# HaydenFaulkner/Tennis

Hardware: AMD Instinct MI355X
Metric: frames/sec DenseNet-121 224x224 feature-extract (higher is better)
Workload: dtype f16

## Files before the change

tennis_amd/csrc/api.hip:

```cpp
#include <cmath>
#include <cstdlib>
#include <cstring>
#include <map>
#include <string>
#include <vector>

#include "common.h"
#include "linear.h"
#include "rnn.h"
#include "train.h"

bool dense_layer_big_supported(int H, int W);

static thread_local std::string g_err;
void tn_set_error(const std::string &msg) { g_err = msg; }
extern "C" const char *tn_last_error(void) { return g_err.c_str(); }
extern "C" int tn_version(void) { return 100; }

extern "C" int tn_ctx_create(int device, void *stream, int own_stream, tn_ctx **out) {
  TN_REQUIRE(out != nullptr, "tn_ctx_create: out is null");
  int n = 0;
  TN_HIP_CHECK(hipGetDeviceCount(&n));
  TN_REQUIRE(device >= 0 && device < n, "tn_ctx_create: no such device");
  TN_ON_DEVICE(device);
// ... 136 lines not shown
          const int n = nf * 16 + (l & 15), slot = (l >> 4) * 8 + j, kx = (slot >> 2) - (zero_first ? 1 : 0), c = slot & 3;
          float v = 0.f;
          if (kx >= 0 && kx < 7 && c < 3) v = w[(((size_t)n * 3 + c) * 7 + ky) * 7 + kx];
          p[(((size_t)ky * 4 + nf) * 64 + l) * 8 + j] = (f16)v;
        }
  return p;
}

struct EventTimer {
  bool on = false;
  hipStream_t s = nullptr;
  struct Rec { hipEvent_t a, b; int fam; };
  std::vector<Rec> recs;
  std::vector<tn_kernel_stat> fams;
  int family(const char *name) {
    for (size_t i = 0; i < fams.size(); ++i)
      if (!strcmp(fams[i].name, name)) return (int)i;
    tn_kernel_stat st;
    memset(&st, 0, sizeof(st));
    strncpy(st.name, name, sizeof(st.name) - 1);
    fams.push_back(st);
    return (int)fams.size() - 1;
  }
  void begin(const char *name, double flops, double bytes) {
    if (!on) return;
    Rec r;
    r.fam = family(name);
    (void)hipEventCreate(&r.a);
    (void)hipEventCreate(&r.b);
    fams[r.fam].launches += 1;
    fams[r.fam].flops += flops;
    fams[r.fam].bytes += bytes;
    (void)hipEventRecord(r.a, s);
    recs.push_back(r);
  }
  void end() {
    if (!on) return;
    (void)hipEventRecord(recs.back().b, s);
  }
  void finish() {
    if (!on) return;
    (void)hipStreamSynchronize(s);
    for (auto &r : recs) {
      float ms = 0.f;
      (void)hipEventElapsedTime(&ms, r.a, r.b);
      fams[r.fam].ms += ms;
      (void)hipEventDestroy(r.a);
      (void)hipEventDestroy(r.b);
    }
    recs.clear();
  }
};

}

struct tn_encoder {
  tn_ctx *ctx;
  DevPool pool;
  int H, W, maxB, feat_dim;
  int Hs, Ws;
  int Hb[4], Wb[4];
  int Cin[4], Cb[4];
  int PH, PW;
  f16 *stem_wp, *stem_wp_zf, *stem_wp_zf_lo = nullptr;
  float *stem_scale, *stem_shift, *stem_shift_u8;
  float *stem_floor = nullptr;
  std::vector<float> stem_centre;
  std::vector<float> calib_centre;
  struct DenseLayer { float *s1, *t1; f16 *w1; float *s2, *t2; f16 *w3p; int cin; f16 *w1s = nullptr, *w3s = nullptr; };
  std::vector<DenseLayer> layers[4];
  struct Trans { float *s, *t; f16 *w; int cin, cout; f16 *wfrag = nullptr; } trans[3];
  float *head_s, *head_t;
  float *zeros128 = nullptr;
  f16 *stem_out, *bott, *blockbuf[4];
  float *head32 = nullptr;
  size_t workspace_bytes;
  int last_batch;
  bool fuse, split;
  int nsplit;
  int dl_variant;
  bool chain;
  bool exact = false;
  bool strip = true;
  int strip_min_batch = 64;
  DenseLayerDev *chain_dev[4] = {nullptr, nullptr, nullptr, nullptr};
  float *calib_dev = nullptr;
  double *calib_scratch = nullptr;
  float *ones128 = nullptr;
  bool block7 = true;
  DenseBlock7Args b7[4] = {};
  bool block14 = true;
  DenseBlock14Args b14[4] = {};
  f16 *b14_scratch[4] = {nullptr, nullptr, nullptr, nullptr};
  bool block28 = false;
  DenseBlock28Args b28[4] = {};
  f16 *b28_scratch[4] = {nullptr, nullptr, nullptr, nullptr};
  hipStream_t side[4];
  hipEvent_t ev_in, ev_done[2][4];
  bool pipelined = false;
  bool last_interleaved = false;
  int last_ws0 = 0;
  bool interleave = false;
  long calls = 0;
  int split_of[2] = {0, 0};
  int split_batch = 0;
};

static const int kBlockCfg[4] = {6, 12, 24, 16};

extern "C" int tn_densenet121_create(tn_ctx *ctx, const tn_param *params, int n_params, const char *prefix_c,
                                     int height, int width, int max_batch, tn_encoder **out) {
  return tn_densenet121_create_ex(ctx, params, n_params, prefix_c, height, width, max_batch, 0, out);
}

extern "C" int tn_densenet121_create_ex(tn_ctx *ctx, const tn_param *params, int n_params, const char *prefix_c,
                                        int height, int width, int max_batch, int flags, tn_encoder **out) {
  TN_REQUIRE(ctx && params && out && prefix_c, "tn_densenet121_create: null argument");
  TN_REQUIRE((flags & ~TN_ENC_EXACT_WEIGHTS) == 0, "tn_densenet121_create_ex: unknown flag");
  TN_REQUIRE(max_batch > 0, "tn_densenet121_create: max_batch must be positive");
  TN_REQUIRE(height >= 224 && width >= 224 && height <= 1024 && width <= 1024,
             "tn_densenet121_create: input size must be in [224,1024] (AvgPool2D(7) needs a >=7x7 final map)");
  TN_ON_DEVICE(ctx->device);
  const std::string pre(prefix_c);
  ParamMap pm(params, n_params);
  tn_encoder *e = new tn_encoder();
  e->ctx = ctx;
  e->H = height; e->W = width; e->maxB = max_batch; e->last_batch = 0;
  e->fuse = getenv("TN_NO_FUSE") == nullptr;
  e->split = getenv("TN_NO_SPLIT") == nullptr;
  e->nsplit = getenv("TN_SPLIT") ? atoi(getenv("TN_SPLIT")) : 2;
  if (e->nsplit != 4) e->nsplit = 2;
  e->block7 = getenv("TN_NO_BLOCK7") == nullptr;
  e->block14 = getenv("TN_NO_BLOCK14") == nullptr;
  e->block28 = getenv("TN_BLOCK28") != nullptr && atoi(getenv("TN_BLOCK28")) != 0;
  e->chain = getenv("TN_NO_CHAIN") == nullptr;
  e->dl_variant = getenv("TN_DL_VARIANT") ? atoi(getenv("TN_DL_VARIANT")) : 0;
  e->exact = (flags & TN_ENC_EXACT_WEIGHTS) != 0;
  e->strip = getenv("TN_NO_STRIP") == nullptr && !e->exact && e->fuse;
  if (getenv("TN_STRIP_MIN_BATCH")) e->strip_min_batch = atoi(getenv("TN_STRIP_MIN_BATCH"));
  for (int i = 0; i < 4; ++i) {
    if (hipStreamCreateWithFlags(&e->side[i], hipStreamNonBlocking) != hipSuccess ||
        hipEventCreateWithFlags(&e->ev_done[0][i], hipEventDisableTiming) != hipSuccess ||
        hipEventCreateWithFlags(&e->ev_done[1][i], hipEventDisableTiming) != hipSuccess) {
      tn_set_error("could not create the side streams");
      delete e;
      return TN_ERR_HIP;
    }
  }
  if (hipEventCreateWithFlags(&e->ev_in, hipEventDisableTiming) != hipSuccess) { tn_set_error("hipEventCreate failed"); delete e; return TN_ERR_HIP; }
  e->Hs = (height + 6 - 7) / 2 + 1; e->Ws = (width + 6 - 7) / 2 + 1;
  int h = (e->Hs + 2 - 3) / 2 + 1, w = (e->Ws + 2 - 3) / 2 + 1, c = 64;
  for (int b = 0; b < 4; ++b) {
    e->Hb[b] = h; e->Wb[b] = w; e->Cin[b] = c; e->Cb[b] = c + 32 * kBlockCfg[b];
    c = e->Cb[b] / 2; h /= 2; w /= 2;
  }
  e->PH = e->Hb[3] / 7; e->PW = e->Wb[3] / 7;
  e->feat_dim = e->Cb[3] * e->PH * e->PW;
  auto fail = [&](int code) { e->pool.release(); delete e; return code; };
  if (e->PH < 1 || e->PW < 1) { tn_set_error("input too small for AvgPool2D(7)"); return fail(TN_ERR_INVALID); }
  if (e->Wb[0] > 240) { tn_set_error("input too wide for the conv3x3 LDS tile"); return fail(TN_ERR_INVALID); }
  if (e->exact) {
    const bool ok = e->fuse && (e->dl_variant & ~256) == 0;
    if (!ok) { tn_set_error("TN_ENC_EXACT_WEIGHTS needs the default kernels (no TN_NO_FUSE, no TN_DL_VARIANT)"); return fail(TN_ERR_INVALID); }
  }

  std::vector<float> s, t;
  e->stem_centre.assign(64, 0.f);
  if (getenv("TN_NO_STEM_CENTRE") == nullptr) {
    std::vector<double> acc(64, 0.0);
    int cnt = 0;
    for (int l = 0; l <= kBlockCfg[0]; ++l) {
      const std::string bn = l < kBlockCfg[0] ? pre + "stage1_batchnorm" + std::to_string(2 * l) : pre + "batchnorm1";
      const float *mu = pm.get(bn + "_running_mean", l < kBlockCfg[0] ? 64 + 32 * l : 64 + 32 * kBlockCfg[0]);
      if (!mu) return fail(TN_ERR_MISSING);
      for (int c = 0; c < 64; ++c) acc[c] += mu[c];
      ++cnt;
    }
    for (int c = 0; c < 64; ++c) {
      const float m = (float)(acc[c] / cnt);
      e->stem_centre[c] = std::isfinite(m) ? m : 0.f;
    }
  }
  auto centre_shift = [&](std::vector<float> &sc, std::vector<float> &sh) {
    for (int c = 0; c < 64; ++c) sh[c] = (float)((double)sh[c] + (double)sc[c] * (double)e->stem_centre[c]);
  };
  {
    const float *w0 = pm.get(pre + "conv0_weight", 64 * 3 * 7 * 7);
    if (!w0 || !fold_bn(pm, pre + "batchnorm0", 64, s, t)) return fail(TN_ERR_MISSING);
    std::vector<float> w0s((size_t)64 * 3 * 49), tu(64);
    for (int n = 0; n < 64; ++n) {
      double bias = 0.0;
      for (int c = 0; c < 3; ++c)
        for (int k = 0; k < 49; ++k) {
          const size_t i = ((size_t)n * 3 + c) * 49 + k;
          w0s[i] = w0[i] * stem_wfactor(c);
          bias -= (double)(float)(f16)w0s[i] * stem_pad(c);
        }
      s[n] = (float)((double)s[n] / kStemWScale);
      tu[n] = (float)((double)t[n] + (double)s[n] * bias);
    }
    e->stem_wp = e->pool.upload(pack_stem(w0s.data(), false));
    e->stem_wp_zf = e->pool.upload(pack_stem(w0s.data(), true));
    if (e->exact) {
      std::vector<float> lo(w0s.size());
      for (int n = 0; n < 64; ++n) {
        double bias = 0.0;
        for (int c = 0; c < 3; ++c)
          for (int k = 0; k < 49; ++k) {
            const size_t i = ((size_t)n * 3 + c) * 49 + k;
            const float hi = (float)(f16)w0s[i];
            lo[i] = w0s[i] - hi;
            bias -= ((double)hi + (double)(float)(f16)lo[i]) * stem_pad(c);
          }
        tu[n] = (float)((double)t[n] + (double)s[n] * bias);
      }
      e->stem_wp_zf_lo = e->pool.upload(pack_stem(lo.data(), true));
    }
    std::vector<float> fl(64);
    for (int n = 0; n < 64; ++n) {
      t[n] = (float)((double)t[n] - (double)e->stem_centre[n]);
      tu[n] = (float)((double)tu[n] - (double)e->stem_centre[n]);
      fl[n] = -e->stem_centre[n];
    }
    e->stem_scale = e->pool.upload(s);
    e->stem_shift = e->pool.upload(t);
    e->stem_shift_u8 = e->pool.upload(tu);
    e->stem_floor = e->pool.upload(fl);
  }
  e->zeros128 = e->pool.upload(std::vector<float>(128, 0.0f));
  e->ones128 = e->pool.upload(std::vector<float>(128, 1.0f));
  int outer = 1;
  for (int b = 0; b < 4; ++b) {
    const std::string sp = pre + "stage" + std::to_string(b + 1) + "_";
    const bool pack14 = e->fuse && e->block14 && !e->exact && dense_block14_supported(e->Hb[b], e->Wb[b], e->Cin[b], kBlockCfg[b]);
    const bool pack28 = e->fuse && e->block28 && !e->exact && dense_block28_supported(e->Hb[b], e->Wb[b], e->Cin[b], kBlockCfg[b]);
    const bool pack7 = (e->fuse && e->block7 && !e->exact && dense_block7_supported(e->Hb[b], e->Wb[b], e->Cin[b], kBlockCfg[b])) || pack14 || pack28;
    std::vector<std::vector<float>> h7[4];
    std::vector<const float *> h7w3;
    for (int l = 0; l < kBlockCfg[b]; ++l) {
      tn_encoder::DenseLayer L;
      L.cin = e->Cin[b] + 32 * l;
      const float *w1 = pm.get(sp + "conv" + std::to_string(2 * l) + "_weight", (int64_t)128 * L.cin);
      const float *w3 = pm.get(sp + "conv" + std::to_string(2 * l + 1) + "_weight", 32 * 128 * 9);
      if (!w1 || !w3) return fail(TN_ERR_MISSING);
      if (!fold_bn(pm, sp + "batchnorm" + std::to_string(2 * l), L.cin, s, t)) return fail(TN_ERR_MISSING);
      if (b == 0) centre_shift(s, t);
      std::vector<float> sw1(L.cin), tc1(L.cin);
      bn_relu_clamp_fold(std::vector<float>(s).data(), std::vector<float>(t).data(), L.cin, s.data(), t.data(), sw1.data(), tc1.data());
      L.s1 = e->pool.upload(s); L.t1 = e->pool.upload(t);
      if (b == 0)
        for (int c = 0; c < 64; ++c) e->calib_centre.push_back(s[c] != t[c] ? e->stem_centre[c] : 0.f);
      std::vector<float> x0(L.cin);
      for (int k = 0; k < L.cin; ++k) x0[k] = std::fmin(std::fmax(0.f, s[k]), t[k]);
      if (pack7) { h7[1].push_back(s); h7[2].push_back(t); h7w3.push_back(w3); }
      if (!fold_bn(pm, sp + "batchnorm" + std::to_string(2 * l + 1), 128, s, t)) return fail(TN_ERR_MISSING);
      std::vector<float> w1f((size_t)128 * L.cin);
      bool in_range = true;
      for (int n = 0; n < 128; ++n) {
        double bias = 0.0, corr = 0.0;
        for (int k = 0; k < L.cin; ++k) {
          const float wf = s[n] * sw1[k] * w1[(size_t)n * L.cin + k];
          w1f[(size_t)n * L.cin + k] = wf;
          in_range = in_range && std::fabs(wf) <= 65504.0f;
          bias += (double)w1[(size_t)n * L.cin + k] * ((double)tc1[k] + (double)sw1[k] * (double)x0[k]);
          if (x0[k] != 0.f) {
            const float hi = (float)(f16)wf;
            const double weff = e->exact ? (double)hi + (double)(float)(f16)(wf - hi) : (double)hi;
            corr += weff * (double)x0[k];
          }
        }
        t[n] = (float)((double)t[n] + (double)s[n] * bias - corr);
      }
      if (!in_range) { tn_set_error("a 1x1 weight leaves the fp16 range once its BatchNorm scales are folded in (" + sp + "conv" + std::to_string(2 * l) + ")"); return fail(TN_ERR_INVALID); }
      if (e->exact) {
        const bool tile = dense_layer_supported(e->Hb[b], e->Wb[b]) && L.cin <= dense_layer_kmax(e->Wb[b]);
        const int bk = !tile ? 64 : (e->Hb[b] == 14 || e->Hb[b] == 7) ? 64 : 32;
        L.w1 = e->pool.upload(split_hi_lo_rows(w1f.data(), 128, L.cin, (L.cin + bk - 1) / bk * bk));
      } else {
        L.w1 = e->pool.upload(to_f16(w1f.data(), (size_t)128 * L.cin));
      }
      if (pack7) { h7[0].push_back(w1f); h7[3].push_back(t); }
      if (e->strip && dense_strip_supported(e->Hb[b], e->Wb[b], L.cin)) L.w1s = e->pool.upload(pack_w1_strip(w1f.data(), L.cin, t.data()));
      L.s2 = e->pool.upload(std::vector<float>(128, 1.0f)); L.t2 = e->pool.upload(t);
      if (e->exact) {
        std::vector<float> hi(32 * 128 * 9), lo(32 * 128 * 9);
        for (size_t i = 0; i < hi.size(); ++i) {
          hi[i] = (float)(f16)w3[i];
          lo[i] = w3[i] - hi[i];
        }
        std::vector<f16> img = pack_conv3x3(hi.data());
        const std::vector<f16> img_lo = pack_conv3x3(lo.data());
        img.insert(img.end(), img_lo.begin(), img_lo.end());
        L.w3p = e->pool.upload(img);
      } else {
        L.w3p = e->pool.upload(pack_conv3x3(w3));
      }
      if (L.w1s) L.w3s = e->pool.upload(pack_w3_strip(w3));
      e->layers[b].push_back(L);
    }
    if (pack14) {
      std::vector<Block14Layer> bl;
      for (int l = 0; l < kBlockCfg[b]; ++l)
        bl.push_back(Block14Layer{h7[0][l].data(), h7w3[l], h7[1][l].data(), h7[2][l].data(), h7[3][l].data()});
      DenseBlock14Args &a14 = e->b14[b];
      a14.stream = e->pool.upload(pack_block14(bl, e->Cin[b]));
      a14.total_units = dense_block14_units(e->Cin[b], kBlockCfg[b]);
      a14.ldc = e->Cb[b]; a14.K0 = e->Cin[b]; a14.nl = kBlockCfg[b];
    } else if (pack28) {
      std::vector<Block14Layer> bl;
      for (int l = 0; l < kBlockCfg[b]; ++l)
        bl.push_back(Block14Layer{h7[0][l].data(), h7w3[l], h7[1][l].data(), h7[2][l].data(), h7[3][l].data()});
      DenseBlock28Args &a28 = e->b28[b];
      a28.stream = e->pool.upload(pack_block28(bl, e->Cin[b]));
      a28.total_units = dense_block28_units(e->Cin[b], kBlockCfg[b]);
      a28.ldc = e->Cb[b]; a28.K0 = e->Cin[b]; a28.nl = kBlockCfg[b];
    } else if (pack7) {
      std::vector<Block7Layer> bl;
      for (int l = 0; l < kBlockCfg[b]; ++l)
        bl.push_back(Block7Layer{h7[0][l].data(), h7w3[l], h7[1][l].data(), h7[2][l].data(), h7[3][l].data()});
      const Block7Image img = pack_block7(bl, e->Cin[b]);
      DenseBlock7Args &a7 = e->b7[b];
      a7.wa = e->pool.upload(img.wa); a7.wb = e->pool.upload(img.wb); a7.tab = e->pool.upload(img.tab);
      for (int w = 0; w < 4; ++w) { a7.a_off[w] = img.a_off[w]; a7.b_off[w] = img.b_off[w]; }
      a7.ldc = e->Cb[b]; a7.K0 = e->Cin[b]; a7.nl = kBlockCfg[b];
    }
    {
      std::vector<DenseLayerDev> cd;
      for (auto &L : e->layers[b]) cd.push_back(DenseLayerDev{L.s1, L.t1, L.w1, L.s2, L.t2, L.w3p});
      e->chain_dev[b] = e->pool.upload(cd);
    }
    if (b < 3) {
      auto &T = e->trans[b];
      T.cin = e->Cb[b]; T.cout = e->Cb[b] / 2;
      const float *wt = pm.get(pre + "conv" + std::to_string(outer) + "_weight", (int64_t)T.cout * T.cin);
      if (!wt || !fold_bn(pm, pre + "batchnorm" + std::to_string(outer), T.cin, s, t)) return fail(TN_ERR_MISSING);
      if (b == 0) centre_shift(s, t);
      T.s = e->pool.upload(s); T.t = e->pool.upload(t);
      T.w = e->exact ? e->pool.upload(split_hi_lo_rows(wt, T.cout, T.cin, T.cin))
                     : e->pool.upload(to_f16(wt, (size_t)T.cout * T.cin));
      if (!e->exact && (T.cout == 512 || T.cout == 256) && T.cin % 128 == 0) {
        const std::vector<f16> wh = to_f16(wt, (size_t)T.cout * T.cin);
        T.wfrag = e->pool.upload(pack_trans_frags(wh.data(), T.cout, T.cin));
      }
      ++outer;
    }
  }
  if (!fold_bn(pm, pre + "batchnorm" + std::to_string(outer), e->Cb[3], s, t)) return fail(TN_ERR_MISSING);
  e->head_s = e->pool.upload(s); e->head_t = e->pool.upload(t);

  const size_t weights_bytes = e->pool.bytes;
  e->interleave = getenv("TN_NO_INTERLEAVE") == nullptr && e->split && max_batch >= 64;
  const size_t B = (size_t)max_batch * (e->interleave ? 2 : 1);
  e->stem_out = (f16 *)e->pool.alloc(B * e->Hs * e->Ws * 64 * sizeof(f16));
  e->bott = (f16 *)e->pool.alloc(B * e->Hb[0] * e->Wb[0] * 128 * sizeof(f16));
  for (int b = 0; b < 4; ++b)
    e->blockbuf[b] = (f16 *)e->pool.alloc(B * e->Hb[b] * e->Wb[b] * e->Cb[b] * sizeof(f16));
  if (e->b7[3].wa) e->head32 = (float *)e->pool.alloc(B * e->Hb[3] * e->Wb[3] * e->Cb[3] * sizeof(float));
  for (int b = 0; b < 4; ++b)
    if (e->b14[b].stream) e->b14_scratch[b] = (f16 *)e->pool.alloc(B * dense_block14_scratch_halfs() * sizeof(f16));
  for (int b = 0; b < 4; ++b)
    if (e->b28[b].stream) e->b28_scratch[b] = (f16 *)e->pool.alloc(B * dense_block28_scratch_halfs() * sizeof(f16));
  e->workspace_bytes = e->pool.bytes - weights_bytes;
  if (e->pool.failed) { tn_set_error("device allocation failed"); return fail(TN_ERR_NOMEM); }
  for (int b = 0; b < 4; ++b)
    if (e->b14[b].stream && (hipMemset(e->blockbuf[b], 0, B * e->Hb[b] * e->Wb[b] * e->Cb[b] * sizeof(f16)) != hipSuccess ||
// ... 653 lines not shown
```

tennis_amd/csrc/dense_strip.hip:

```cpp
#include <array>
#include <vector>

#include "common.h"

int launch_dense_strip_w56(const DenseStripArgs &a, hipStream_t s);
int launch_dense_strip_w28(const DenseStripArgs &a, hipStream_t s);
int launch_dense_strip_w128(const DenseStripArgs &a, hipStream_t s);
int launch_dense_strip_w64(const DenseStripArgs &a, hipStream_t s);

bool dense_strip_supported(int H, int W, int K) {
  return H == W && (W == 56 || W == 28 || W == 128 || W == 64) && K % 32 == 0 && K >= 64 && K <= (W == 128 ? 288 : 320);
}

int launch_dense_strip(const DenseStripArgs &a, hipStream_t s) {
  TN_REQUIRE(dense_strip_supported(a.H, a.W, a.K), "dense_strip: unsupported geometry");
  TN_REQUIRE(a.buf && a.s1 && a.t1 && a.w1s && a.w3s, "dense_strip: null operand");
  TN_REQUIRE(a.ldc % 64 == 0 && a.K + 32 <= a.ldc, "dense_strip: bad channel geometry");
  if (a.W == 56) return launch_dense_strip_w56(a, s);
  if (a.W == 128) return launch_dense_strip_w128(a, s);
  if (a.W == 64) return launch_dense_strip_w64(a, s);
  return launch_dense_strip_w28(a, s);
}

std::vector<f16> pack_w1_strip(const float *w, int K, const float *shift) {
  const int ks = K / 32, kq = K / 16, nsu = (ks + 1) / 2;
  std::vector<f16> p((size_t)(kq + 1) * 4 * 64 * 8, (f16)0.f);
  for (int mb = 0; mb < 4; ++mb)
    for (int l = 0; l < 32; ++l) {
      f16 *d = &p[(((size_t)kq * 4 + mb) * 64 + l) * 8];
      const float t = shift[32 * mb + l];
      d[0] = (f16)t;
      d[1] = (f16)(t - (float)d[0]);
      d[2] = (f16)1.f;
    }
  for (int q = 0; q < kq; ++q) {
    const int u = q >> 2, i = q & 3;
    const bool half = (ks & 1) && u == nsu - 1;
    for (int mb = 0; mb < 4; ++mb)
      for (int l = 0; l < 64; ++l)
        for (int j = 0; j < 8; ++j) {
          const int c = (half ? 64 * u + 16 * (l >> 5) : 64 * u + 32 * (l >> 5)) + 8 * i + j;
          p[(((size_t)q * 4 + mb) * 64 + l) * 8 + j] = (f16)w[(size_t)(32 * mb + (l & 31)) * K + c];
        }
  }
  return p;
}

std::vector<f16> pack_w3_strip(const float *w) {
  constexpr int kW3Bytes = 3 * 8 * 3 * 1024;
  std::vector<f16> p((size_t)kW3Bytes / 2);
  for (int dy = 0; dy < 3; ++dy)
    for (int t = 0; t < 8; ++t)
      for (int dx = 0; dx < 3; ++dx)
        for (int l = 0; l < 64; ++l)
          for (int j = 0; j < 8; ++j) {
            const int m = l & 31, o = 16 * ((m >> 2) & 1) + (m & 3) + 4 * (m >> 3);
            const int c = 16 * t + 8 * (j >> 2) + 4 * (l >> 5) + (j & 3);
            p[(((((size_t)dy * 8 + t) * 3 + dx) * 64) + l) * 8 + j] = (f16)w[(((size_t)o * 128 + c) * 3 + dy) * 3 + dx];
          }
  return p;
}
```

tennis_amd/csrc/dense_strip_impl.h:

```cpp
#include <array>
#include <type_traits>

#pragma once
#include "common.h"

#ifndef TN_DS_EXP
#define TN_DS_EXP 0
#endif

namespace {

typedef unsigned u32x4 __attribute__((ext_vector_type(4)));
typedef _Float16 h2_t __attribute__((ext_vector_type(2)));

constexpr int kW3Bytes = 3 * 8 * 3 * 1024;

template <int W, int KS>
struct DSGeom {
  static constexpr int NPAIR = (W + 27) / 28;
  static constexpr int ROWS = W == 56 ? 28 : W == 28 ? 7 : W / 4;
  static constexpr int NCHUNK = W / ROWS;
  static constexpr int NITEM = NPAIR * NCHUNK, WGS = NITEM / 4;
  static constexpr int KQ = 2 * KS;
  static constexpr int NSU = (KS + 1) / 2;
  static constexpr int W1OFF = kW3Bytes;
  static constexpr int T1OFF = W1OFF + (KQ + 1) * 4096;
  static constexpr int LDS_BYTES = T1OFF + KS * 32 * 4;
  static_assert(W % ROWS == 0 && NITEM % 4 == 0 && ROWS >= 4, "strip geometry");
  static_assert(NSU <= 5, "the activation ring holds five super-steps");
  static_assert(LDS_BYTES <= 160 * 1024, "weights do not fit LDS");
};

#define TN_WIN_BASE 160
#define TN_WIN_CLOBBER                                                                                                              \
  "a160", "a161", "a162", "a163", "a164", "a165", "a166", "a167", "a168", "a169", "a170", "a171", "a172", "a173", "a174", "a175",   \
  "a176", "a177", "a178", "a179", "a180", "a181", "a182", "a183", "a184", "a185", "a186", "a187", "a188", "a189", "a190", "a191",   \
  "a192", "a193", "a194", "a195", "a196", "a197", "a198", "a199", "a200", "a201", "a202", "a203", "a204", "a205", "a206", "a207",   \
  "a208", "a209", "a210", "a211", "a212", "a213", "a214", "a215", "a216", "a217", "a218", "a219", "a220", "a221", "a222", "a223",   \
  "a224", "a225", "a226", "a227", "a228", "a229", "a230", "a231", "a232", "a233", "a234", "a235", "a236", "a237", "a238", "a239",   \
  "a240", "a241", "a242", "a243", "a244", "a245", "a246", "a247", "a248", "a249", "a250", "a251", "a252", "a253", "a254", "a255"
constexpr int win_reg(int prow, int t) { return TN_WIN_BASE + 32 * prow + 4 * t; }
#define TN_WIN_FENCE() asm volatile("" ::: TN_WIN_CLOBBER)

template <int PROW, int T>
__device__ __forceinline__ void win_write(const unsigned v0, const unsigned v1, const unsigned v2, const unsigned v3) {
  constexpr int B = win_reg(PROW, T);
  asm volatile("v_accvgpr_write_b32 a%c4, %0\n\tv_accvgpr_write_b32 a%c5, %1\n\tv_accvgpr_write_b32 a%c6, %2\n\tv_accvgpr_write_b32 a%c7, %3"
               :: "v"(v0), "v"(v1), "v"(v2), "v"(v3), "n"(B), "n"(B + 1), "n"(B + 2), "n"(B + 3) : TN_WIN_CLOBBER);
}
template <int R>
__device__ __forceinline__ void win_zero_reg() {
  asm volatile("v_accvgpr_write_b32 a%c0, 0" :: "n"(R) : TN_WIN_CLOBBER);
}
template <int PROW>
__device__ __forceinline__ void win_zero() {
  [&]<int... I>(std::integer_sequence<int, I...>) { (win_zero_reg<win_reg(PROW, 0) + I>(), ...); }(std::make_integer_sequence<int, 32>{});
  asm volatile("s_nop 1");
}
template <bool FIRST, int PROW, int T>
__device__ __forceinline__ void mfma32_win(f32x16 &d, const u32x4 a) {
  constexpr int B0 = win_reg(PROW, T);
  if constexpr (FIRST)
    asm volatile("v_mfma_f32_32x32x16_f16 %0, %1, a[%c2:%c3], 0" : "=&a"(d) : "v"(a), "n"(B0), "n"(B0 + 3));
  else
    asm volatile("v_mfma_f32_32x32x16_f16 %0, %1, a[%c2:%c3], %0" : "+a"(d) : "v"(a), "n"(B0), "n"(B0 + 3));
}
template <int PROW, int T>
__device__ __forceinline__ void mfma32_win_last3(f32x16 &d0, f32x16 &d1, f32x16 &d2, const u32x4 a0, const u32x4 a1, const u32x4 a2) {
  constexpr int B0 = win_reg(PROW, T);
  asm volatile("v_mfma_f32_32x32x16_f16 %0, %3, a[%c6:%c7], %0\n\tv_mfma_f32_32x32x16_f16 %1, %4, a[%c6:%c7], %1\n\t"
               "v_mfma_f32_32x32x16_f16 %2, %5, a[%c6:%c7], %2\n\ts_nop 15\n\ts_nop 3"
               : "+a"(d0), "+a"(d1), "+a"(d2) : "v"(a0), "v"(a1), "v"(a2), "n"(B0), "n"(B0 + 3));
}
__device__ __forceinline__ f32x16 mfma32(const u32x4 a, const u32x4 b, const f32x16 c) {
  return __builtin_amdgcn_mfma_f32_32x32x16_f16(__builtin_bit_cast(f16x8, a), __builtin_bit_cast(f16x8, b), c, 0, 0, 0);
}

template <int CTRL>
__device__ __forceinline__ float dpp_f32(float v) {
  return __builtin_bit_cast(float, __builtin_amdgcn_update_dpp(0, __builtin_bit_cast(int, v), CTRL, 0xf, 0xf, true));
}

#define TN_INL __attribute__((always_inline))
template <int N, typename F>
__device__ __forceinline__ void static_for(F &&f) {
  [&]<int... I>(std::integer_sequence<int, I...>) TN_INL { (f(std::integral_constant<int, I>{}), ...); }(std::make_integer_sequence<int, N>{});
}
template <int V>
using ic = std::integral_constant<int, V>;

#define TN_SB() __builtin_amdgcn_sched_barrier(0)

__device__ __forceinline__ void dma16(const void *gsrc, unsigned lds_dst) {
  unsigned keep;
  asm volatile("s_mov_b32 %0, m0\n\ts_mov_b32 m0, %2\n\ts_nop 0\n\tglobal_load_lds_dwordx4 %1, off\n\ts_mov_b32 m0, %0"
               : "=&s"(keep)
               : "v"(gsrc), "s"(lds_dst)
               : "memory");
}

struct PItem { int kind, q, j; };
template <int KS>
struct PList { PItem it[7 * 2 * KS + 8]; int n; };
template <int KS>
constexpr PList<KS> make_pl() {
  constexpr int KQ = 2 * KS, NSU = (KS + 1) / 2;
  constexpr bool ODD = (KS & 1) != 0;
  PList<KS> l{};
  int n = 0;
  for (int c = 0; c < 3 && c < KQ; ++c) l.it[n++] = PItem{1, c, 0};
  for (int q = 0; q < KQ; ++q) {
    for (int j = 0; j < 4; ++j) l.it[n++] = PItem{2, q, j};
    if (q + 3 < KQ) l.it[n++] = PItem{1, q + 3, 0};
    const int u = q >> 2;
    const bool half = ODD && u == NSU - 1;
    if (half ? (q & 3) == 1 : (q & 3) == 3)
      for (int i = 0; i < (half ? 2 : 4); ++i) l.it[n++] = PItem{3, u, i};
  }
  l.n = n;
  return l;
}
template <int KS>
inline constexpr PList<KS> kPL = make_pl<KS>();
template <int KS>
constexpr PItem pl_at(int idx) { return idx >= 0 && idx < kPL<KS>.n ? kPL<KS>.it[idx] : PItem{0, 0, 0}; }
template <int KS>
constexpr int pl_len() { return kPL<KS>.n; }
constexpr int kPLB = 30;
constexpr int kXN = 8;
struct ASlot { int pl0, npl, epb0, nepb; };
template <int N> struct ASched { ASlot s[N]; };
template <int KS>
constexpr auto make_a_sched() {
  constexpr int KQ = 2 * KS, NA = 4 * (KQ + 1), NPL = pl_len<KS>();
  ASched<NA> r{};
  int bn3[KQ + 1] = {};
  for (int i = 0; i < NPL; ++i)
    if (kPL<KS>.it[i].kind == 2 && kPL<KS>.it[i].j == 3) bn3[kPL<KS>.it[i].q] = i;
  int pos = NPL < kPLB ? NPL : kPLB, epb = 0;
  for (int i = 0; i < NA; ++i) {
    const int qn = i / 4 + 1, rem = 3 - i % 4;
    const int need_end = qn < KQ ? bn3[qn] + 1 : 0;
    const int left = NA - i, total = (NPL - pos) + (24 - epb);
    int quota = (total + left - 1) / left;
    int must = need_end - rem - pos;
    if (must < 0) must = 0;
    if (must > NPL - pos) must = NPL - pos;
    int npl = must;
    if (quota < npl) quota = npl;
    int ne = 24 - epb < quota - npl ? 24 - epb : quota - npl;
    const int more = NPL - pos - npl < quota - npl - ne ? NPL - pos - npl : quota - npl - ne;
    npl += more;
    r.s[i] = ASlot{pos, npl, epb, ne};
    pos += npl;
    epb += ne;
  }
  return r;
}
template <int KS>
constexpr bool a_sched_complete() {
  constexpr int KQ = 2 * KS, NA = 4 * (KQ + 1);
  constexpr auto sa = make_a_sched<KS>();
  int npl = pl_len<KS>() < kPLB ? pl_len<KS>() : kPLB, nepb = 0;
  for (int i = 0; i < NA; ++i) { npl += sa.s[i].npl; nepb += sa.s[i].nepb; }
  return npl == pl_len<KS>() && nepb == 24;
}

template <int W, int KS>
__global__ __launch_bounds__(256) __attribute__((amdgpu_waves_per_eu(1, 1))) void dense_strip_kernel(DenseStripArgs a) {
  using G = DSGeom<W, KS>;
  constexpr int H = W, NSU = G::NSU, K = KS * 32, KQ = G::KQ, ROWS = G::ROWS;
  constexpr bool ODD = (KS & 1) != 0;
  constexpr int XN = kXN, NPL = pl_len<KS>(), PLB = NPL < kPLB ? NPL : kPLB;
  static_assert(a_sched_complete<KS>(), "1x1 slot schedule leaves work unassigned");
  extern __shared__ __attribute__((aligned(16))) unsigned char smem[];
  const int tid = threadIdx.x;
  if (a.ts && tid == 0) {
    a.ts[(size_t)blockIdx.x * 128 + 127] = __builtin_amdgcn_s_memtime();
    a.ts[(size_t)blockIdx.x * 128 + 126] = __builtin_amdgcn_s_memrealtime();
  }

  {
    typedef __attribute__((address_space(3))) void *lptr_t;
    const unsigned lds0 = __builtin_amdgcn_readfirstlane((unsigned)(size_t)(lptr_t)smem);
    const int wv = __builtin_amdgcn_readfirstlane(tid >> 6), ln = tid & 63;
    constexpr int P3 = kW3Bytes / 1024, P1 = (KQ + 1) * 4;
    const unsigned char *g3 = (const unsigned char *)a.w3s + ln * 16, *g1 = (const unsigned char *)a.w1s + ln * 16;
    for (int p = wv; p < P3; p += 4) dma16(g3 + p * 1024, lds0 + p * 1024);
    for (int p = wv; p < P1; p += 4) dma16(g1 + p * 1024, lds0 + G::W1OFF + p * 1024);
    f16 *t1 = (f16 *)(smem + G::T1OFF);
    for (int i = tid; i < K; i += 256) {
      t1[i] = (f16)a.s1[i];
      t1[K + i] = (f16)a.t1[i];
    }
    asm volatile("s_waitcnt vmcnt(0)" ::: "memory");
  }
  __syncthreads();

  const int lane = tid & 63;
  const int wid = __builtin_amdgcn_readfirstlane(tid >> 6);
  const int n = lane & 31, h = lane >> 5;
  const int item = (int)(blockIdx.x % G::WGS) * 4 + wid;
  const int pair = item % G::NPAIR, part = item / G::NPAIR;
  const int r_lo = part * ROWS, r_hi = r_lo + ROWS;
  const int x = 14 * (2 * pair + (n >> 4)) - 1 + (n & 15);
  const bool xvalid = x >= 0 && x < W;
  const int xc = x < 0 ? 0 : (x >= W ? W - 1 : x);
  const int ldc = a.ldc;
  const unsigned rowpitch = (unsigned)W * ldc * 2;
  unsigned char *fb = (unsigned char *)(a.buf + (size_t)(blockIdx.x / G::WGS) * H * W * ldc);
  const unsigned colb = (unsigned)xc * ldc * 2 + 64 * h;
  const unsigned colh = (unsigned)xc * ldc * 2 + 32 * h;
  const bool store_ok = (n & 15) >= 1 && (n & 15) <= 14 && xvalid;
  const unsigned outb = (unsigned)xc * ldc * 2 + K * 2 + 32 * h;
  const __amdgpu_buffer_rsrc_t orsrc = __builtin_amdgcn_make_buffer_rsrc(fb, 0, (int)((unsigned)H * rowpitch), 0x00020000);

  const unsigned char *w1l = smem + G::W1OFF + lane * 16;
  const unsigned char *w3l = smem + lane * 16;
  const f16 *tab1 = (const f16 *)(smem + G::T1OFF);
  const u32x4 xb_shift = {h == 0 ? 0x3c003c00u : 0u, (h == 0 && !xvalid) ? 0x0000fb53u : 0u, 0u, 0u};

  u32x4 ring[5][4];
  f32x16 acc[4];
  u32x4 wa[2][4];
  u32x4 xb[XN];
  u32x4 cs[3], ct[3];
  u32x4 w3f[2][3];
  f32x16 bacc[3];
  unsigned e_pk[4];
  float o_c[2], o_l[2], o_r[2];
  unsigned o_pk[8];

  auto rowbase = [&](int y) TN_INL {
    const int yc = y < 0 ? 0 : (y >= H ? H - 1 : y);
    return fb + (unsigned)yc * rowpitch;
  };
  auto ld_item = [&](auto u_tag, auto i_tag, int y) TN_INL {
    constexpr int U = decltype(u_tag)::value, I = decltype(i_tag)::value;
    constexpr bool HALF = ODD && U == NSU - 1;
    if ((TN_DS_EXP & 1) && y > r_lo + 1) return;
    if constexpr (HALF) ring[U][I] = *(const u32x4 *)(rowbase(y) + colh + 128 * U + 16 * I);
    else ring[U][I] = *(const u32x4 *)(rowbase(y) + colb + 128 * U + 16 * I);
  };
  auto consts_item = [&](auto q_tag) TN_INL {
    constexpr int Q = decltype(q_tag)::value;
    constexpr int U = Q >> 2, I = Q & 3;
    constexpr bool HALF = ODD && U == NSU - 1;
    const int c0 = (HALF ? 64 * U + 16 * h : 64 * U + 32 * h) + 8 * I;
    cs[Q % 3] = *(const u32x4 *)(tab1 + c0);
    ct[Q % 3] = *(const u32x4 *)(tab1 + K + c0);
  };
  auto bn_item = [&](auto q_tag, auto j_tag) TN_INL {
    constexpr int Q = decltype(q_tag)::value, J = decltype(j_tag)::value;
    const unsigned in = ring[Q >> 2][Q & 3][J];
    const unsigned sc = cs[Q % 3][J], sh = ct[Q % 3][J];
    unsigned o;
    asm("v_pk_max_f16 %0, %1, %2\n\tv_pk_min_f16 %0, %0, %3" : "=&v"(o) : "v"(in), "v"(sc), "v"(sh));
    xb[Q % XN][J] = o;
  };
  auto pl_item = [&](auto idx_tag, int ybn) TN_INL {
    constexpr PItem it = pl_at<KS>(decltype(idx_tag)::value);
    if constexpr (it.kind == 1) consts_item(ic<it.q>{});
    else if constexpr (it.kind == 2) bn_item(ic<it.q>{}, ic<it.j>{});
    else if constexpr (it.kind == 3) ld_item(ic<it.q>{}, ic<it.j>{}, ybn + 1);
  };
  auto wa_item = [&](auto q_tag, auto mb_tag) TN_INL {
    constexpr int Q = decltype(q_tag)::value, MB = decltype(mb_tag)::value;
    if ((TN_DS_EXP & 16) && Q >= 2) return;
    wa[Q & 1][MB] = *(const u32x4 *)(w1l + (Q * 4 + MB) * 1024);
  };
  auto wa_group = [&](auto q_tag) TN_INL { static_for<4>([&](auto mb_tag) TN_INL { wa_item(q_tag, mb_tag); }); };
  auto prologue_exposed = [&](int ybn) TN_INL {
    wa_group(ic<0>{});
    wa_group(ic<1>{});
    static_for<PLB>([&](auto i_tag) TN_INL { pl_item(i_tag, ybn); });
    TN_SB();
  };

  auto epa_item = [&](auto prow_tag, auto e_tag) TN_INL {
    constexpr int PROW = decltype(prow_tag)::value, E = decltype(e_tag)::value;
    constexpr int T = E / 5, I = E % 5, MB = T >> 1, R0 = 8 * (T & 1);
    unsigned (&epk)[4] = e_pk;
    f32x16 (&accr)[4] = acc;
    if constexpr (I < 4) {
      const float a0 = accr[MB][R0 + 2 * I], a1 = accr[MB][R0 + 2 * I + 1];
      asm("v_cvt_pk_f16_f32 %0, %1, %2\n\tv_pk_max_f16 %0, %0, 0" : "=v"(epk[I]) : "v"(a0), "v"(a1));
    } else {
      win_write<PROW, T>(epk[0], epk[1], epk[2], epk[3]);
    }
  };
  auto epilogue_a_exposed = [&](auto prow_tag) TN_INL {
    static_for<40>([&](auto e_tag) TN_INL { epa_item(prow_tag, e_tag); });
    TN_SB();
  };
  auto epb_item = [&](auto i_tag, unsigned off) TN_INL {
    constexpr int I = decltype(i_tag)::value, P = I / 3, PART = I % 3;
    if constexpr (PART == 0) {
      o_c[0] = bacc[1][2 * P]; o_c[1] = bacc[1][2 * P + 1];
      o_l[0] = bacc[0][2 * P]; o_l[1] = bacc[0][2 * P + 1];
    } else if constexpr (PART == 1) {
      o_c[0] += dpp_f32<0x111>(o_l[0]);
      o_c[1] += dpp_f32<0x111>(o_l[1]);
      o_r[0] = bacc[2][2 * P]; o_r[1] = bacc[2][2 * P + 1];
    } else {
      o_c[0] += dpp_f32<0x101>(o_r[0]);
      o_c[1] += dpp_f32<0x101>(o_r[1]);
      const h2_t p = {(f16)o_c[0], (f16)o_c[1]};
      o_pk[P] = __builtin_bit_cast(unsigned, p);
      if constexpr (P == 3 || P == 7) {
        const u32x4 o = {o_pk[P - 3], o_pk[P - 2], o_pk[P - 1], o_pk[P]};
        __builtin_amdgcn_raw_buffer_store_b128(o, orsrc, off + (P == 7 ? 16 : 0), 0, 0);
      }
    }
  };
  auto out_offset = [&](int yo, bool valid) TN_INL { return (valid && store_ok) ? outb + (unsigned)yo * rowpitch : 0x80000000u; };
  auto bacc_ready = [&]() TN_INL {
    f32x16 (&b)[3] = bacc;
    asm volatile("s_nop 15\n\ts_nop 3" : "+a"(b[0]), "+a"(b[1]), "+a"(b[2]));
  };
  auto epilogue_b_exposed = [&](int yo) TN_INL {
    bacc_ready();
    const unsigned off = out_offset(yo, true);
    static_for<24>([&](auto i_tag) TN_INL { epb_item(i_tag, off); TN_SB(); });
  };
  auto w3_item = [&](auto s_tag, auto dx_tag) TN_INL {
    constexpr int S = decltype(s_tag)::value, DX = decltype(dx_tag)::value;
    if ((TN_DS_EXP & 8) && S >= 2) return;
    w3f[S & 1][DX] = *(const u32x4 *)(w3l + (S * 3 + DX) * 1024);
  };

  auto phase_a = [&](int yb, int yo_prev, bool prev_valid) TN_INL {
    constexpr auto SA = make_a_sched<KS>();
    bacc_ready();
    const unsigned off_prev = out_offset(yo_prev, prev_valid);
    static_for<KQ + 1>([&](auto q_tag) TN_INL {
      constexpr int Q = decltype(q_tag)::value;
      static_for<4>([&](auto mb_tag) TN_INL {
        constexpr int MB = decltype(mb_tag)::value, SL = 4 * Q + MB;
        if constexpr (MB == 0) {
          u32x4 (&w)[4] = wa[Q & 1];
          asm volatile("" :: "v"(w[0]), "v"(w[1]), "v"(w[2]), "v"(w[3]));
        }
        if constexpr (Q == 0) {
          f32x16 z;
#pragma unroll
          for (int i = 0; i < 16; ++i) z[i] = 0.f;
          acc[MB] = mfma32(wa[0][MB], xb[0], z);
        } else if constexpr (Q == KQ) {
          acc[MB] = mfma32(wa[Q & 1][MB], xb_shift, acc[MB]);
        } else {
          acc[MB] = mfma32(wa[Q & 1][MB], xb[Q % XN], acc[MB]);
        }
        if constexpr (Q + 2 < KQ + 1) wa_item(ic<Q + 2>{}, mb_tag);
        constexpr ASlot sl = SA.s[SL];
        static_for<sl.npl>([&](auto k_tag) TN_INL { pl_item(ic<sl.pl0 + decltype(k_tag)::value>{}, yb); });
        static_for<sl.nepb>([&](auto k_tag) TN_INL { epb_item(ic<sl.epb0 + decltype(k_tag)::value>{}, off_prev); });
        TN_WIN_FENCE();
        TN_SB();
      });
    });
  };

  auto phase_b = [&](auto rot_tag, auto epa_tag, int ybn) TN_INL {
    constexpr int ROT = decltype(rot_tag)::value;
    constexpr bool HAS_EPA = decltype(epa_tag)::value != 0;
    static_for<72>([&](auto e_tag) TN_INL {
      constexpr int E = decltype(e_tag)::value;
      constexpr int S = E / 3, DX = E % 3, DY = S / 8, T = S % 8;
      constexpr int PROW = (ROT + 1 + DY) % 3;
      if constexpr (DX == 0) {
        u32x4 (&w)[3] = w3f[S & 1];
        asm volatile("" :: "v"(w[0]), "v"(w[1]), "v"(w[2]));
      }
      if constexpr (S < 23) mfma32_win<S == 0, PROW, T>(bacc[DX], w3f[S & 1][DX]);
      else if constexpr (DX == 2) mfma32_win_last3<PROW, T>(bacc[0], bacc[1], bacc[2], w3f[S & 1][0], w3f[S & 1][1], w3f[S & 1][2]);
      if constexpr (S + 2 < 24) w3_item(ic<S + 2>{}, ic<DX>{});
      if constexpr (E < 40) {
        if constexpr (HAS_EPA) epa_item(rot_tag, e_tag);
      } else if constexpr (E < 42) {
        wa_group(ic<E - 40>{});
      } else if constexpr (E - 42 < PLB) {
        pl_item(ic<E - 42>{}, ybn);
      }
      TN_WIN_FENCE();
      TN_SB();
    });
  };
  auto load_w3_first = [&]() TN_INL { static_for<6>([&](auto i_tag) TN_INL { w3_item(ic<decltype(i_tag)::value / 3>{}, ic<decltype(i_tag)::value % 3>{}); }); };

  int nstamp = 0;
  auto stamp = [&]() TN_INL {
    if (a.ts && wid == 0 && nstamp < 125) {
      if (lane == 0) a.ts[(size_t)blockIdx.x * 128 + nstamp] = __builtin_amdgcn_s_memtime();
      ++nstamp;
    }
  };
  auto row_event = [&](auto rot_tag, int yb, bool prev_valid) TN_INL {
    stamp();
    if (!(TN_DS_EXP & 4)) phase_a(yb, yb - 2, prev_valid);
    load_w3_first();
    TN_SB();
    stamp();
    if (!(TN_DS_EXP & 2)) phase_b(rot_tag, ic<1>{}, yb + 1);
  };

  {
    f32x16 z;
#pragma unroll
    for (int i = 0; i < 16; ++i) z[i] = 0.f;
    bacc[0] = z; bacc[1] = z; bacc[2] = z;
  }
  stamp();
  const int yfirst = r_lo > 0 ? r_lo - 1 : 0;
  static_for<NSU>([&](auto u_tag) TN_INL {
    constexpr bool HALF = ODD && decltype(u_tag)::value == NSU - 1;
    static_for<(HALF ? 2 : 4)>([&](auto i_tag) TN_INL { ring[decltype(u_tag)::value][decltype(i_tag)::value] =
        *(const u32x4 *)(rowbase(yfirst) + (HALF ? colh : colb) + 128 * decltype(u_tag)::value + 16 * decltype(i_tag)::value); });
  });
  if (r_lo > 0) {
    prologue_exposed(r_lo - 1);
    phase_a(r_lo - 1, 0, false);
    epilogue_a_exposed(ic<0>{});
  } else {
    win_zero<0>();
  }
  prologue_exposed(r_lo);
  phase_a(r_lo, 0, false);
  epilogue_a_exposed(ic<1>{});
  prologue_exposed(r_lo + 1);
  stamp();
  int yb = r_lo + 1;
  for (; yb + 2 < r_hi; yb += 3) {
    row_event(ic<2>{}, yb, yb > r_lo + 1);
    row_event(ic<0>{}, yb + 1, true);
    row_event(ic<1>{}, yb + 2, true);
  }
  constexpr int NREM = (ROWS - 1) % 3;
  if constexpr (NREM >= 1) { row_event(ic<2>{}, yb, yb > r_lo + 1); ++yb; }
  if constexpr (NREM >= 2) { row_event(ic<0>{}, yb, true); ++yb; }
  constexpr int ROTL = (ROWS + 1) % 3;
  if (r_hi < H) {
    row_event(ic<ROTL>{}, r_hi, true);
  } else {
    epilogue_b_exposed(r_hi - 2);
    win_zero<ROTL>();
    load_w3_first();
    TN_SB();
    phase_b(ic<ROTL>{}, ic<0>{}, r_hi);
  }
  stamp();
  epilogue_b_exposed(r_hi - 1);
  stamp();
  if (a.ts && wid == 0 && lane == 0) a.ts[(size_t)blockIdx.x * 128 + 125] = __builtin_amdgcn_s_memrealtime();
}

template <int W, int KS>
int launch_strip(const DenseStripArgs &a, hipStream_t s) {
  using G = DSGeom<W, KS>;
  TN_SET_ATTR_ONCE_PER_DEVICE(TN_HIP_CHECK(hipFuncSetAttribute((const void *)dense_strip_kernel<W, KS>, hipFuncAttributeMaxDynamicSharedMemorySize, G::LDS_BYTES)));
  hipLaunchKernelGGL((dense_strip_kernel<W, KS>), dim3(a.B * G::WGS), dim3(256), G::LDS_BYTES, s, a);
  TN_HIP_CHECK(hipGetLastError());
  return TN_OK;
}

template <int W>
int launch_strip_w(const DenseStripArgs &a, hipStream_t s) {
  switch (a.K / 32) {
    case 2: return launch_strip<W, 2>(a, s);
    case 3: return launch_strip<W, 3>(a, s);
    case 4: return launch_strip<W, 4>(a, s);
    case 5: return launch_strip<W, 5>(a, s);
    case 6: return launch_strip<W, 6>(a, s);
    case 7: return launch_strip<W, 7>(a, s);
    case 8: return launch_strip<W, 8>(a, s);
    case 9: return launch_strip<W, 9>(a, s);
    case 10:
      if constexpr (W != 128) return launch_strip<W, 10>(a, s);
      break;
  }
  TN_REQUIRE(false, "dense_strip: K out of range");
}

}
```

Measured before the change: 134,200.

## Extend fused strip dense-layer kernel to wider 28x28 inputs via global-memory weight tail

Lets the fused 1x1+3x3 strip kernel handle 28x28 dense layers with up to 480 input channels. When the 1x1 weights no longer fit in LDS, the first k-steps stay LDS-resident and the rest are streamed from global memory with buffer loads. The activation ring is re-indexed modulo a shorter depth, and a third weight register slot is added for small tails. Layers that previously fell back to the slower unfused path now run fused, at the cost of more global weight traffic and register pressure in those instances.

```diff
diff --git a/tennis_amd/csrc/api.hip b/tennis_amd/csrc/api.hip
--- a/tennis_amd/csrc/api.hip
+++ b/tennis_amd/csrc/api.hip
@@ -242,6 +242,7 @@
   bool chain;
   bool exact = false;
   bool strip = true;
+  int strip_kmax = 480;
   int strip_min_batch = 64;
   DenseLayerDev *chain_dev[4] = {nullptr, nullptr, nullptr, nullptr};
   float *calib_dev = nullptr;
@@ -298,6 +299,7 @@
   e->exact = (flags & TN_ENC_EXACT_WEIGHTS) != 0;
   e->strip = getenv("TN_NO_STRIP") == nullptr && !e->exact && e->fuse;
   if (getenv("TN_STRIP_MIN_BATCH")) e->strip_min_batch = atoi(getenv("TN_STRIP_MIN_BATCH"));
+  if (getenv("TN_STRIP_KMAX")) e->strip_kmax = atoi(getenv("TN_STRIP_KMAX"));
   for (int i = 0; i < 4; ++i) {
     if (hipStreamCreateWithFlags(&e->side[i], hipStreamNonBlocking) != hipSuccess ||
         hipEventCreateWithFlags(&e->ev_done[0][i], hipEventDisableTiming) != hipSuccess ||
@@ -440,7 +442,7 @@
         L.w1 = e->pool.upload(to_f16(w1f.data(), (size_t)128 * L.cin));
       }
       if (pack7) { h7[0].push_back(w1f); h7[3].push_back(t); }
-      if (e->strip && dense_strip_supported(e->Hb[b], e->Wb[b], L.cin)) L.w1s = e->pool.upload(pack_w1_strip(w1f.data(), L.cin, t.data()));
+      if (e->strip && L.cin <= e->strip_kmax && dense_strip_supported(e->Hb[b], e->Wb[b], L.cin)) L.w1s = e->pool.upload(pack_w1_strip(w1f.data(), L.cin, t.data()));
       L.s2 = e->pool.upload(std::vector<float>(128, 1.0f)); L.t2 = e->pool.upload(t);
       if (e->exact) {
         std::vector<float> hi(32 * 128 * 9), lo(32 * 128 * 9);
diff --git a/tennis_amd/csrc/dense_strip.hip b/tennis_amd/csrc/dense_strip.hip
--- a/tennis_amd/csrc/dense_strip.hip
+++ b/tennis_amd/csrc/dense_strip.hip
@@ -5,11 +5,13 @@
 
 int launch_dense_strip_w56(const DenseStripArgs &a, hipStream_t s);
 int launch_dense_strip_w28(const DenseStripArgs &a, hipStream_t s);
+int launch_dense_strip_w28_tail(const DenseStripArgs &a, hipStream_t s);
 int launch_dense_strip_w128(const DenseStripArgs &a, hipStream_t s);
 int launch_dense_strip_w64(const DenseStripArgs &a, hipStream_t s);
 
 bool dense_strip_supported(int H, int W, int K) {
-  return H == W && (W == 56 || W == 28 || W == 128 || W == 64) && K % 32 == 0 && K >= 64 && K <= (W == 128 ? 288 : 320);
+  return H == W && (W == 56 || W == 28 || W == 128 || W == 64) && K % 32 == 0 && K >= 64 &&
+         K <= (W == 128 ? 288 : W == 28 ? 480 : 320);
 }
 
 int launch_dense_strip(const DenseStripArgs &a, hipStream_t s) {
@@ -19,7 +21,7 @@
   if (a.W == 56) return launch_dense_strip_w56(a, s);
   if (a.W == 128) return launch_dense_strip_w128(a, s);
   if (a.W == 64) return launch_dense_strip_w64(a, s);
-  return launch_dense_strip_w28(a, s);
+  return a.K > 320 ? launch_dense_strip_w28_tail(a, s) : launch_dense_strip_w28(a, s);
 }
 
 std::vector<f16> pack_w1_strip(const float *w, int K, const float *shift) {
diff --git a/tennis_amd/csrc/dense_strip_impl.h b/tennis_amd/csrc/dense_strip_impl.h
--- a/tennis_amd/csrc/dense_strip_impl.h
+++ b/tennis_amd/csrc/dense_strip_impl.h
@@ -14,6 +14,12 @@
 typedef _Float16 h2_t __attribute__((ext_vector_type(2)));
 
 constexpr int kW3Bytes = 3 * 8 * 3 * 1024;
+
+constexpr int strip_nqr(int ks) {
+  const int fit = (160 * 1024 - kW3Bytes - ks * 32 * 4) / 4096;
+  return 2 * ks + 1 < fit ? 2 * ks + 1 : fit;
+}
+constexpr int strip_dq(int ks) { return strip_nqr(ks) < 2 * ks + 1 ? ks : 2 * ks; }
 
 template <int W, int KS>
 struct DSGeom {
@@ -23,11 +29,16 @@
   static constexpr int NITEM = NPAIR * NCHUNK, WGS = NITEM / 4;
   static constexpr int KQ = 2 * KS;
   static constexpr int NSU = (KS + 1) / 2;
+  static constexpr int NQR = strip_nqr(KS);
+  static constexpr bool TAIL = NQR < KQ + 1;
+  static constexpr int DQ = strip_dq(KS);
+  static constexpr int NWA = TAIL && KS < 15 ? 3 : 2;
   static constexpr int W1OFF = kW3Bytes;
-  static constexpr int T1OFF = W1OFF + (KQ + 1) * 4096;
+  static constexpr int T1OFF = W1OFF + NQR * 4096;
   static constexpr int LDS_BYTES = T1OFF + KS * 32 * 4;
   static_assert(W % ROWS == 0 && NITEM % 4 == 0 && ROWS >= 4, "strip geometry");
-  static_assert(NSU <= 5, "the activation ring holds five super-steps");
+  static_assert(DQ <= 20, "the activation ring holds at most twenty k-steps");
+  static_assert(!TAIL || NQR >= 4, "the first k-steps of the 1x1 are LDS-resident (the 3x3 phase preloads k-steps 0 .. NWA - 1)");
   static_assert(LDS_BYTES <= 160 * 1024, "weights do not fit LDS");
 };
 
@@ -101,11 +112,11 @@
 
 struct PItem { int kind, q, j; };
 template <int KS>
-struct PList { PItem it[7 * 2 * KS + 8]; int n; };
+struct PList { PItem it[7 * 2 * KS + 8]; int n, nd; };
 template <int KS>
 constexpr PList<KS> make_pl() {
-  constexpr int KQ = 2 * KS, NSU = (KS + 1) / 2;
-  constexpr bool ODD = (KS & 1) != 0;
+  constexpr int KQ = 2 * KS, NSU = (KS + 1) / 2, DQ = strip_dq(KS);
+  constexpr bool ODD = (KS & 1) != 0, TAIL = DQ < KQ;
   PList<KS> l{};
   int n = 0;
   for (int c = 0; c < 3 && c < KQ; ++c) l.it[n++] = PItem{1, c, 0};
@@ -114,9 +125,14 @@
     if (q + 3 < KQ) l.it[n++] = PItem{1, q + 3, 0};
     const int u = q >> 2;
     const bool half = ODD && u == NSU - 1;
-    if (half ? (q & 3) == 1 : (q & 3) == 3)
+    if ((half ? (q & 3) == 1 : (q & 3) == 3) && !(TAIL && 4 * u >= DQ))
       for (int i = 0; i < (half ? 2 : 4); ++i) l.it[n++] = PItem{3, u, i};
   }
+  l.nd = n;
+  if (TAIL)
+    for (int u = 0; u < NSU; ++u)
+      if (4 * u >= DQ)
+        for (int i = 0; i < (ODD && u == NSU - 1 ? 2 : 4); ++i) l.it[n++] = PItem{3, u, i};
   l.n = n;
   return l;
 }
@@ -132,7 +148,7 @@
 template <int N> struct ASched { ASlot s[N]; };
 template <int KS>
 constexpr auto make_a_sched() {
-  constexpr int KQ = 2 * KS, NA = 4 * (KQ + 1), NPL = pl_len<KS>();
+  constexpr int KQ = 2 * KS, NA = 4 * (KQ + 1), NPL = pl_len<KS>(), ND = kPL<KS>.nd;
   ASched<NA> r{};
   int bn3[KQ + 1] = {};
   for (int i = 0; i < NPL; ++i)
@@ -141,15 +157,16 @@
   for (int i = 0; i < NA; ++i) {
     const int qn = i / 4 + 1, rem = 3 - i % 4;
     const int need_end = qn < KQ ? bn3[qn] + 1 : 0;
+    const int cap = i < 4 * (KQ - 1) ? ND : NPL;
     const int left = NA - i, total = (NPL - pos) + (24 - epb);
     int quota = (total + left - 1) / left;
     int must = need_end - rem - pos;
     if (must < 0) must = 0;
-    if (must > NPL - pos) must = NPL - pos;
+    if (must > cap - pos) must = cap - pos;
     int npl = must;
     if (quota < npl) quota = npl;
     int ne = 24 - epb < quota - npl ? 24 - epb : quota - npl;
-    const int more = NPL - pos - npl < quota - npl - ne ? NPL - pos - npl : quota - npl - ne;
+    const int more = cap - pos - npl < quota - npl - ne ? cap - pos - npl : quota - npl - ne;
     npl += more;
     r.s[i] = ASlot{pos, npl, epb, ne};
     pos += npl;
@@ -169,7 +186,7 @@
 template <int W, int KS>
 __global__ __launch_bounds__(256) __attribute__((amdgpu_waves_per_eu(1, 1))) void dense_strip_kernel(DenseStripArgs a) {
   using G = DSGeom<W, KS>;
-  constexpr int H = W, NSU = G::NSU, K = KS * 32, KQ = G::KQ, ROWS = G::ROWS;
+  constexpr int H = W, NSU = G::NSU, K = KS * 32, KQ = G::KQ, ROWS = G::ROWS, DQ = G::DQ, NQR = G::NQR, NWA = G::NWA;
   constexpr bool ODD = (KS & 1) != 0;
   constexpr int XN = kXN, NPL = pl_len<KS>(), PLB = NPL < kPLB ? NPL : kPLB;
   static_assert(a_sched_complete<KS>(), "1x1 slot schedule leaves work unassigned");
@@ -184,7 +201,7 @@
     typedef __attribute__((address_space(3))) void *lptr_t;
     const unsigned lds0 = __builtin_amdgcn_readfirstlane((unsigned)(size_t)(lptr_t)smem);
     const int wv = __builtin_amdgcn_readfirstlane(tid >> 6), ln = tid & 63;
-    constexpr int P3 = kW3Bytes / 1024, P1 = (KQ + 1) * 4;
+    constexpr int P3 = kW3Bytes / 1024, P1 = NQR * 4;
     const unsigned char *g3 = (const unsigned char *)a.w3s + ln * 16, *g1 = (const unsigned char *)a.w1s + ln * 16;
     for (int p = wv; p < P3; p += 4) dma16(g3 + p * 1024, lds0 + p * 1024);
     for (int p = wv; p < P1; p += 4) dma16(g1 + p * 1024, lds0 + G::W1OFF + p * 1024);
@@ -216,13 +233,14 @@
   const __amdgpu_buffer_rsrc_t orsrc = __builtin_amdgcn_make_buffer_rsrc(fb, 0, (int)((unsigned)H * rowpitch), 0x00020000);
 
   const unsigned char *w1l = smem + G::W1OFF + lane * 16;
+  const __amdgpu_buffer_rsrc_t w1rsrc = __builtin_amdgcn_make_buffer_rsrc((void *)a.w1s, 0, (KQ + 1) * 4096, 0x00020000);
   const unsigned char *w3l = smem + lane * 16;
   const f16 *tab1 = (const f16 *)(smem + G::T1OFF);
   const u32x4 xb_shift = {h == 0 ? 0x3c003c00u : 0u, (h == 0 && !xvalid) ? 0x0000fb53u : 0u, 0u, 0u};
 
   u32x4 ring[5][4];
   f32x16 acc[4];
-  u32x4 wa[2][4];
+  u32x4 wa[NWA][4];
   u32x4 xb[XN];
   u32x4 cs[3], ct[3];
   u32x4 w3f[2][3];
@@ -235,12 +253,18 @@
     const int yc = y < 0 ? 0 : (y >= H ? H - 1 : y);
     return fb + (unsigned)yc * rowpitch;
   };
-  auto ld_item = [&](auto u_tag, auto i_tag, int y) TN_INL {
-    constexpr int U = decltype(u_tag)::value, I = decltype(i_tag)::value;
+  auto ld_step = [&](auto t_tag, int y) TN_INL {
+    constexpr int T = decltype(t_tag)::value, U = T >> 2, I = T & 3;
     constexpr bool HALF = ODD && U == NSU - 1;
-    if ((TN_DS_EXP & 1) && y > r_lo + 1) return;
-    if constexpr (HALF) ring[U][I] = *(const u32x4 *)(rowbase(y) + colh + 128 * U + 16 * I);
-    else ring[U][I] = *(const u32x4 *)(rowbase(y) + colb + 128 * U + 16 * I);
+    constexpr int S = T % DQ;
+    if constexpr (HALF) ring[S >> 2][S & 3] = *(const u32x4 *)(rowbase(y) + colh + 128 * U + 16 * I);
+    else ring[S >> 2][S & 3] = *(const u32x4 *)(rowbase(y) + colb + 128 * U + 16 * I);
+  };
+  auto ld_item = [&](auto u_tag, auto i_tag, int ybn) TN_INL {
+    constexpr int T = 4 * decltype(u_tag)::value + decltype(i_tag)::value + DQ;
+    if ((TN_DS_EXP & 1) && ybn + (T >= KQ) > r_lo + 1) return;
+    if constexpr (T < KQ) ld_step(ic<T>{}, ybn);
+    else ld_step(ic<T - KQ>{}, ybn + 1);
   };
   auto consts_item = [&](auto q_tag) TN_INL {
     constexpr int Q = decltype(q_tag)::value;
@@ -252,7 +276,7 @@
   };
   auto bn_item = [&](auto q_tag, auto j_tag) TN_INL {
     constexpr int Q = decltype(q_tag)::value, J = decltype(j_tag)::value;
-    const unsigned in = ring[Q >> 2][Q & 3][J];
+    const unsigned in = ring[(Q % DQ) >> 2][(Q % DQ) & 3][J];
     const unsigned sc = cs[Q % 3][J], sh = ct[Q % 3][J];
     unsigned o;
     asm("v_pk_max_f16 %0, %1, %2\n\tv_pk_min_f16 %0, %0, %3" : "=&v"(o) : "v"(in), "v"(sc), "v"(sh));
@@ -262,17 +286,18 @@
     constexpr PItem it = pl_at<KS>(decltype(idx_tag)::value);
     if constexpr (it.kind == 1) consts_item(ic<it.q>{});
     else if constexpr (it.kind == 2) bn_item(ic<it.q>{}, ic<it.j>{});
-    else if constexpr (it.kind == 3) ld_item(ic<it.q>{}, ic<it.j>{}, ybn + 1);
+    else if constexpr (it.kind == 3) ld_item(ic<it.q>{}, ic<it.j>{}, ybn);
   };
   auto wa_item = [&](auto q_tag, auto mb_tag) TN_INL {
     constexpr int Q = decltype(q_tag)::value, MB = decltype(mb_tag)::value;
     if ((TN_DS_EXP & 16) && Q >= 2) return;
-    wa[Q & 1][MB] = *(const u32x4 *)(w1l + (Q * 4 + MB) * 1024);
+    if ((TN_DS_EXP & 32) && Q >= NQR) return;
+    if constexpr (Q < NQR) wa[Q % NWA][MB] = *(const u32x4 *)(w1l + (Q * 4 + MB) * 1024);
+    else wa[Q % NWA][MB] = __builtin_bit_cast(u32x4, __builtin_amdgcn_raw_buffer_load_b128(w1rsrc, lane * 16, (Q * 4 + MB) * 1024, 0));
   };
   auto wa_group = [&](auto q_tag) TN_INL { static_for<4>([&](auto mb_tag) TN_INL { wa_item(q_tag, mb_tag); }); };
   auto prologue_exposed = [&](int ybn) TN_INL {
-    wa_group(ic<0>{});
-    wa_group(ic<1>{});
+    static_for<NWA>([&](auto q_tag) TN_INL { wa_group(q_tag); });
     static_for<PLB>([&](auto i_tag) TN_INL { pl_item(i_tag, ybn); });
     TN_SB();
   };
@@ -338,7 +363,7 @@
       static_for<4>([&](auto mb_tag) TN_INL {
         constexpr int MB = decltype(mb_tag)::value, SL = 4 * Q + MB;
         if constexpr (MB == 0) {
-          u32x4 (&w)[4] = wa[Q & 1];
+          u32x4 (&w)[4] = wa[Q % NWA];
           asm volatile("" :: "v"(w[0]), "v"(w[1]), "v"(w[2]), "v"(w[3]));
         }
         if constexpr (Q == 0) {
@@ -347,11 +372,11 @@
           for (int i = 0; i < 16; ++i) z[i] = 0.f;
           acc[MB] = mfma32(wa[0][MB], xb[0], z);
         } else if constexpr (Q == KQ) {
-          acc[MB] = mfma32(wa[Q & 1][MB], xb_shift, acc[MB]);
+          acc[MB] = mfma32(wa[Q % NWA][MB], xb_shift, acc[MB]);
         } else {
-          acc[MB] = mfma32(wa[Q & 1][MB], xb[Q % XN], acc[MB]);
+          acc[MB] = mfma32(wa[Q % NWA][MB], xb[Q % XN], acc[MB]);
         }
-        if constexpr (Q + 2 < KQ + 1) wa_item(ic<Q + 2>{}, mb_tag);
+        if constexpr (Q + NWA < KQ + 1) wa_item(ic<Q + NWA>{}, mb_tag);
         constexpr ASlot sl = SA.s[SL];
         static_for<sl.npl>([&](auto k_tag) TN_INL { pl_item(ic<sl.pl0 + decltype(k_tag)::value>{}, yb); });
         static_for<sl.nepb>([&](auto k_tag) TN_INL { epb_item(ic<sl.epb0 + decltype(k_tag)::value>{}, off_prev); });
@@ -379,6 +404,7 @@
         if constexpr (HAS_EPA) epa_item(rot_tag, e_tag);
       } else if constexpr (E < 42) {
         wa_group(ic<E - 40>{});
+        if constexpr (E == 41 && NWA == 3) wa_group(ic<2>{});
       } else if constexpr (E - 42 < PLB) {
         pl_item(ic<E - 42>{}, ybn);
       }
@@ -412,11 +438,7 @@
   }
   stamp();
   const int yfirst = r_lo > 0 ? r_lo - 1 : 0;
-  static_for<NSU>([&](auto u_tag) TN_INL {
-    constexpr bool HALF = ODD && decltype(u_tag)::value == NSU - 1;
-    static_for<(HALF ? 2 : 4)>([&](auto i_tag) TN_INL { ring[decltype(u_tag)::value][decltype(i_tag)::value] =
-        *(const u32x4 *)(rowbase(yfirst) + (HALF ? colh : colb) + 128 * decltype(u_tag)::value + 16 * decltype(i_tag)::value); });
-  });
+  static_for<DQ>([&](auto t_tag) TN_INL { ld_step(t_tag, yfirst); });
   if (r_lo > 0) {
     prologue_exposed(r_lo - 1);
     phase_a(r_lo - 1, 0, false);
diff --git a/tennis_amd/csrc/dense_strip_w28k.hip b/tennis_amd/csrc/dense_strip_w28k.hip
--- /dev/null
+++ b/tennis_amd/csrc/dense_strip_w28k.hip
@@ -0,0 +1,12 @@
+#include "dense_strip_impl.h"
+
+int launch_dense_strip_w28_tail(const DenseStripArgs &a, hipStream_t s) {
+  switch (a.K / 32) {
+    case 11: return launch_strip<28, 11>(a, s);
+    case 12: return launch_strip<28, 12>(a, s);
+    case 13: return launch_strip<28, 13>(a, s);
+    case 14: return launch_strip<28, 14>(a, s);
+    case 15: return launch_strip<28, 15>(a, s);
+  }
+  TN_REQUIRE(false, "dense_strip: K out of range");
+}
```

Result: no change. 134,200 (median of 6 runs) (+0.0%).
